# Mephisto405/WCMC

Hardware: AMD Instinct MI355X
Metric: 128x128 MC patches/sec (train step), KPCN-Manifold (higher is better)
Workload: dtype bf16x321h

## Files before the change

### include/wcmc_hip.h

```cpp
#ifndef WCMC_HIP_H
#define WCMC_HIP_H

#include <stddef.h>
#include <stdint.h>

#ifdef __cplusplus
extern "C" {
#endif

#define WCMC_ABI_VERSION 2

enum wcmc_status {
  WCMC_OK = 0,
  WCMC_ERR_BAD_ARG = -1,
  WCMC_ERR_ALIGNMENT = -2,
  WCMC_ERR_WORKSPACE = -3,
  WCMC_ERR_LAUNCH = -4
};

enum wcmc_act { WCMC_ACT_LINEAR = 0, WCMC_ACT_RELU = 1, WCMC_ACT_LEAKY_RELU = 2 };

int wcmc_abi_version(void);
const char* wcmc_last_error(void);

// ... 76 lines not shown
int wcmc_embed3_mean_fwd(const void* x_split, int64_t M, int Cin, const void* wp0, const float* b0, const void* wp1,
                         const float* b1, const void* wp2, const float* b2, float* y, float* y_mean, int S, int64_t HW,
                         void* stream);
int wcmc_embed3_bwd(const void* x_split, int64_t M, int Cin, const void* wp0, const float* b0, const void* wp1,
                    const float* b1, const void* wt1, const void* wt2, const float* gy, int gy_pixel_stride,
                    const float* gm, int gm_pixel_stride, int S, int64_t HW, float gm_scale, float* dw0, float* db0,
                    float* dw1, float* db1, float* dw2, float* db2, void* workspace, size_t workspace_bytes, void* stream);
int wcmc_final2_supported(int C1, int C2, int Chid, int outc, int64_t HW);
size_t wcmc_final2_bwd_workspace_bytes(void);
int wcmc_final2_fwd(const float* y, int y_pixel_stride, const float* prop, int prop_pixel_stride, int B, int S, int64_t HW,
                    const void* wp0, const float* b0, const void* wp1, const float* b1, int outc, float* out, void* stream);
int wcmc_final2_bwd(const float* y, int y_pixel_stride, const float* prop, int prop_pixel_stride, int B, int S, int64_t HW,
                    const void* wp0, const float* b0, const void* wp1, const float* b1, int outc, const void* wt0,
                    const void* wt1, const float* gout, float* dy, float* dprop, float* dw0, float* db0, float* dw1,
                    float* db1, void* workspace, size_t workspace_bytes, void* stream);
size_t wcmc_conv2d_igemm_colsum_elems(int N, int Ho, int Wo, int Cout);
int wcmc_colsum_finish(const float* partial, int N, int Ho, int Wo, int Cout, float* db, void* stream);
int wcmc_conv2d_launch_plan_bf16x3(int N, int H, int W, int Cin, int Cout, int ks, int pad, int terms, int split_out,
                                   int64_t ysn, int64_t ysh, int64_t ysw, int gate_tensor, int out_f16,
                                   char* cls, char* kernel, size_t len);
int wcmc_conv2d_wgrad_launch_plan_bf16x3(int N, int H, int W, int Cin, int Cout, int ks, int pad, int terms,
                                         char* cls, char* kernel, size_t len);
size_t wcmc_conv2d_wgrad_bf16x3_workspace_bytes(int N, int Ho, int Wo, int Cout, int Cin, int ks);
int wcmc_conv2d_wgrad_reduce_multi(int n, void* const* workspace, float* const* dw, float* const* db,
                                   const float* const* dy_colsum_partial, const int* N, const int* Ho, const int* Wo,
                                   const int* Cout, const int* Cin, const int* ks, int terms, void* stream);
int wcmc_conv2d_wgrad_bf16x3(const void* x_split, int N, int H, int W, int Cin,
                             const void* dy_split, int Cout, int ks, int pad, float* dw, float* db,
                             void* workspace, size_t workspace_bytes, int phase, const float* dy_colsum_partial,
                             int terms, void* stream);
// ... 233 lines not shown
```

### wcmc_amd/_lib.py

```python
import ctypes
import os

_HERE = os.path.dirname(os.path.abspath(__file__))
LIB_PATH = os.path.join(_HERE, "libwcmc_hip.so")
if os.environ.get("WCMC_DEBUG_LIB") == "1":
    LIB_PATH = os.path.join(_HERE, "libwcmc_hip_debug.so")
if os.environ.get("WCMC_LIB_AB"):
    LIB_PATH = os.path.join(_HERE, os.path.basename(os.environ["WCMC_LIB_AB"]))

_c = ctypes
P, I, L, F, D, Z = _c.c_void_p, _c.c_int, _c.c_int64, _c.c_float, _c.c_double, _c.c_size_t

SIGNATURES = {
    "wcmc_abi_version": (I, []),
    "wcmc_last_error": (_c.c_char_p, []),
    "wcmc_to_nhwc": (I, [P, L, L, L, L, P, L, L, L, I, I, I, I, P]),
    "wcmc_from_nhwc": (I, [P, L, L, L, P, L, L, L, L, I, I, I, I, P]),
    "wcmc_conv2d_packed_elems": (Z, [I, I, I]),
    "wcmc_conv2d_pack_weight": (I, [P, P, I, I, I, I, P]),
    "wcmc_conv2d_igemm": (I, [P, L, L, L, I, I, I, I, P, P, P, L, L, L, I, I, I, I, F,
                              P, L, L, L, I, F, P]),
    "wcmc_conv2d_wgrad_workspace_bytes": (Z, [I, I, I, I, I, I]),
    "wcmc_conv2d_wgrad": (I, [P, L, L, L, I, I, I, I, P, L, L, L, I, I, I, P, P, P, Z, P]),
    "wcmc_split_elems": (Z, [I, I, I, I]),
# ... 47 lines not shown
    "wcmc_pbuffer_cat_fwd": (I, [P, L, L, L, L, P, L, L, L, L, L, P, L, L, L, I, I, I, I, I, I, P]),
    "wcmc_pbuffer_cat_bwd": (I, [P, L, L, L, P, L, L, L, L, L, I, I, I, I, I, I, P]),
    "wcmc_feature_mse_workspace_bytes": (Z, [I, I, I, I, I]),
    "wcmc_feature_mse_fwd": (I, [P, L, L, L, L, L, P, L, L, L, L, P, P, P, P, Z, I, I, I, I, I, P]),
    "wcmc_feature_mse_bwd": (I, [P, L, L, L, L, L, P, P, P, P, P, Z, I, I, I, I, I, P]),
    "wcmc_grs_fwd": (I, [P, L, L, L, L, L, P, L, L, L, L, P, P, F, P, P, Z, I, I, I, I, I, P]),
    "wcmc_grs_bwd": (I, [P, L, L, L, L, L, P, P, P, P, P, Z, I, I, I, I, I, P]),
    "wcmc_random_permutation": (I, [P, L, ctypes.c_uint64, P]),
    "wcmc_permutation_key": (ctypes.c_uint64, [ctypes.c_uint64, ctypes.c_uint64, I]),
    "wcmc_random_permutation_dev": (I, [P, L, P, I, P]),
    "wcmc_step_counter_advance": (I, [P, P]),
    "wcmc_final2_supported": (I, [I, I, I, I, L]),
    "wcmc_final2_bwd_workspace_bytes": (Z, []),
    "wcmc_final2_fwd": (I, [P, I, P, I, I, I, L, P, P, P, P, I, P, P]),
    "wcmc_final2_bwd": (I, [P, I, P, I, I, I, L, P, P, P, P, I, P, P, P, P, P, P, P, P, P, P, Z, P]),
    "wcmc_embed3_supported": (I, [I, I, I, I]),
    "wcmc_embed3_bwd_workspace_bytes": (Z, []),
    "wcmc_embed3_fwd": (I, [P, L, I, P, P, P, P, P, P, P, P]),
    "wcmc_embed3_mean_supported": (I, [I, L]),
    "wcmc_embed3_mean_fwd": (I, [P, L, I, P, P, P, P, P, P, P, P, I, L, P]),
    "wcmc_embed3_bwd": (I, [P, L, I, P, P, P, P, P, P, P, I, P, I, I, L, F, P, P, P, P, P, P, P, Z, P]),
    "wcmc_image_loss2_fwd": (I, [I, P, L, L, L, L, P, L, L, L, L, F, P, P, Z, I, I, I, I, P]),
    "wcmc_image_loss2_bwd": (I, [I, P, L, L, L, L, P, L, L, L, L, F, P, P, I, I, I, I, P]),
    "wcmc_grad_norm_clip_workspace_bytes": (Z, [I, P]),
    "wcmc_grad_norm_clip": (I, [I, P, P, F, P, P, Z, P]),
    "wcmc_weight_norm_fwd": (I, [I, P, P, P, P, P, P, P]),
    "wcmc_weight_norm_bwd": (I, [I, P, P, P, P, P, P, P, P, P]),
    "wcmc_clip_adam": (I, [P, P, P, P, L, F, D, D, D, D, I, F, P, P]),
    "wcmc_clip_adam_hyper": (None, [D, D, D, D, I, P]),
    "wcmc_clip_adam_dev": (I, [P, P, P, P, L, F, F, P, P, P]),
# ... 61 lines not shown
```

### wcmc_amd/csrc/pathnet_fused.hip

```cpp
#include <stdlib.h>

#include "common.h"

namespace wcmc {

typedef __bf16 bf16x8 __attribute__((ext_vector_type(8)));
typedef unsigned short u16;
typedef short s16x4 __attribute__((ext_vector_type(4)));
typedef unsigned u32x2 __attribute__((ext_vector_type(2)));
typedef unsigned u32x4 __attribute__((ext_vector_type(4)));

constexpr unsigned E3_OOB = 0x80000000u;
constexpr int E3_TP = 64;
constexpr int E3_C = 64;
constexpr int E3_RS = 80;
constexpr int E3_TILE = E3_TP * E3_RS;

__device__ __forceinline__ u16 e3_bf(float x) { return __builtin_bit_cast(u16, (__bf16)x); }
__device__ __forceinline__ float e3_f(u16 h) { return __builtin_bit_cast(float, (unsigned)h << 16); }
__device__ __forceinline__ float e3_u2f(unsigned v) { return __builtin_bit_cast(float, v); }
__device__ __forceinline__ unsigned e3_f2u(float v) { return __builtin_bit_cast(unsigned, v); }

struct E3Params {
  const u16* x; int64_t M; int Cp0, Kt0;
// ... 371 lines not shown
}

constexpr int F2_C = 128;
constexpr int F2_RS = 144;
constexpr int F2_TILE = E3_TP * F2_RS;
constexpr int F2_ORS = 48;
constexpr int F2_W1RS = 2 * 128 + 8;

struct F2Params {
  const float* y; int y_ps;
  const float* prop; int p_ps;
  int B, S; int64_t HW;
  const u16* wp0; const u16* wp1;
  const float* b0; const float* b1; int outc;
  float* out; int os;
  const u16* wt0; const u16* wt1;
  const float* gout;
  float* dy; float* dprop;
  float* ws;
  unsigned y_bytes, p_bytes, o_bytes, dy_bytes, dp_bytes;
};
constexpr int F2_WS_PER_BLOCK = F2_C * F2_C + 16 * F2_C + F2_C + 16;

struct F2W { bf16x8 h[4], l[4]; };
__device__ __forceinline__ F2W f2_load_w(const u16* wp, int row, int q) {
  F2W w;
#pragma unroll
  for (int c = 0; c < 4; ++c) {
    const u16* a = wp + (int64_t)(row * 2) * F2_C + c * 32 + q * 8;
    w.h[c] = *reinterpret_cast<const bf16x8*>(a);
// ... 60 lines not shown
  for (int i = 0; i < 4; ++i) {
    u16 hi[4], lo[4];
#pragma unroll
    for (int e = 0; e < 4; ++e) {
      const float t = acc[i][e] + b[e];
      const float v = t > 0.f ? t : 0.f;
      hi[e] = e3_bf(v);
      lo[e] = e3_bf(v - e3_f(hi[e]));
    }
    const int o = (16 * i + fr) * F2_RS + 16 * wave + 4 * q;
    *reinterpret_cast<u32x2*>(th + o) = u32x2{(unsigned)hi[0] | ((unsigned)hi[1] << 16), (unsigned)hi[2] | ((unsigned)hi[3] << 16)};
    *reinterpret_cast<u32x2*>(tl + o) = u32x2{(unsigned)lo[0] | ((unsigned)lo[1] << 16), (unsigned)lo[2] | ((unsigned)lo[3] << 16)};
  }
}

template <bool BWD>
__global__ __launch_bounds__(512, 1) void final2_kernel(F2Params p) {
  extern __shared__ __attribute__((aligned(16))) u16 lds[];
  u16* const CH = lds; u16* const CL = lds + F2_TILE; u16* const HH = lds + 2 * F2_TILE; u16* const HL = lds + 3 * F2_TILE;
  u16* const DHH = lds + 4 * F2_TILE;
  u16* const DOH = lds + 5 * F2_TILE;
  float* const stg = reinterpret_cast<float*>(HL);
  float* const red = reinterpret_cast<float*>(lds + 5 * F2_TILE + E3_TP * F2_ORS);
  const int tid = threadIdx.x, lane = tid & 63, wave = tid >> 6, fr = lane & 15, q = lane >> 4;
  const __amdgpu_buffer_rsrc_t yr = __builtin_amdgcn_make_buffer_rsrc((void*)p.y, 0, (int)p.y_bytes, 0x00020000);
  const __amdgpu_buffer_rsrc_t pr = __builtin_amdgcn_make_buffer_rsrc((void*)p.prop, 0, (int)p.p_bytes, 0x00020000);
  const __amdgpu_buffer_rsrc_t orr = __builtin_amdgcn_make_buffer_rsrc((void*)(BWD ? (void*)p.gout : (void*)p.out), 0, (int)p.o_bytes, 0x00020000);
  u16* const W1S = reinterpret_cast<u16*>(red + 16 * F2_C + 64 * 8);
  const F2W w0 = f2_load_w(p.wp0, 16 * wave + fr, q);
  F2W w1;
  if (!BWD) w1 = f2_load_w(p.wp1, fr, q);
  float b0[4], b1[4];
#pragma unroll
  for (int e = 0; e < 4; ++e) { b0[e] = p.b0[16 * wave + 4 * q + e]; b1[e] = (4 * q + e < p.outc) ? p.b1[4 * q + e] : 0.f; }
  const int oq = p.os >> 2;
  const int64_t tpi = p.HW / E3_TP;
  const int64_t nsuper = (int64_t)p.B * tpi;

  F2W t0;
  bf16x8 t1h, t1l;
  f32x4 gw0[8], gw1;
  float sb0[4] = {0.f, 0.f, 0.f, 0.f}, sb1[4] = {0.f, 0.f, 0.f, 0.f};
// ... 20 lines not shown
    f32x4 dpacc[4];
#pragma unroll
    for (int i = 0; i < 4; ++i) dpacc[i] = f32x4{0.f, 0.f, 0.f, 0.f};
    for (int s = 0; s < p.S; ++s) {
      const int64_t m0 = (b * p.S + s) * p.HW + hw0;
      f2_store64_split(yp, CH, CL, 0, tid);
      u32x4 go = {0u, 0u, 0u, 0u};
      if (BWD && wave < 4 && q < oq)
        go = __builtin_amdgcn_raw_buffer_load_b128(orr, (unsigned)(m0 * p.os * 4) + (unsigned)((16 * wave + fr) * p.os * 4 + q * 16), 0, 0);
      if (s + 1 < p.S) yp = f2_load64(yr, (b * p.S + s + 1) * p.HW + hw0, p.y_ps, tid);
      __syncthreads();
      f32x4 acc[4];
      f2_gemm<3, 4>(acc, w0, CH, CL, 0, fr, q);
      f2_store_relu_split(acc, b0, HH, HL, wave, fr, q);
      __syncthreads();
      float ov[4] = {0.f, 0.f, 0.f, 0.f};
      if (wave < 4) {
        f32x4 a2[1];
        if (BWD) {
          a2[0] = f32x4{0.f, 0.f, 0.f, 0.f};
#pragma unroll
          for (int c = 0; c < 4; ++c) {
            const int o = (16 * wave + fr) * F2_RS + c * 32 + q * 8;
            const bf16x8 ah = *reinterpret_cast<const bf16x8*>(HH + o), al = *reinterpret_cast<const bf16x8*>(HL + o);
            const bf16x8 wh = *reinterpret_cast<const bf16x8*>(W1S + fr * F2_W1RS + c * 32 + q * 8);
            const bf16x8 wl = *reinterpret_cast<const bf16x8*>(W1S + fr * F2_W1RS + F2_C + c * 32 + q * 8);
            a2[0] = __builtin_amdgcn_mfma_f32_16x16x32_bf16(wl, ah, a2[0], 0, 0, 0);
            a2[0] = __builtin_amdgcn_mfma_f32_16x16x32_bf16(wh, al, a2[0], 0, 0, 0);
            a2[0] = __builtin_amdgcn_mfma_f32_16x16x32_bf16(wh, ah, a2[0], 0, 0, 0);
          }
// ... 65 lines not shown
        const int v = tid + 512 * k, px = v >> 4, c4 = (v & 15) * 4;
        const float4 o = *reinterpret_cast<const float4*>(stg + px * 68 + c4);
        const u32x4 o4 = {__builtin_bit_cast(unsigned, o.x), __builtin_bit_cast(unsigned, o.y), __builtin_bit_cast(unsigned, o.z),
                          __builtin_bit_cast(unsigned, o.w)};
        __builtin_amdgcn_raw_buffer_store_b128(o4, dyr, (unsigned)(m0 * 256) + (unsigned)(px * 256 + c4 * 4), 0, 0);
      }
    }
    if (BWD && wave >= 4) {
#pragma unroll
      for (int i = 0; i < 4; ++i) {
        const u32x4 o4 = {e3_f2u(dpacc[i][0]), e3_f2u(dpacc[i][1]), e3_f2u(dpacc[i][2]), e3_f2u(dpacc[i][3])};
        __builtin_amdgcn_raw_buffer_store_b128(o4, dpr, (unsigned)((b * p.HW + hw0) * 256) + (unsigned)((16 * i + fr) * 256 + (16 * (wave - 4) + 4 * q) * 4), 0, 0);
      }
    }
  }
  if (!BWD) return;
  float* ws = p.ws + (int64_t)blockIdx.x * F2_WS_PER_BLOCK;
#pragma unroll
  for (int j = 0; j < 8; ++j)
#pragma unroll
    for (int e = 0; e < 4; ++e) ws[(16 * wave + 4 * q + e) * F2_C + 16 * j + fr] = gw0[j][e];
#pragma unroll
  for (int e = 0; e < 4; ++e) ws[F2_C * F2_C + (4 * q + e) * F2_C + 16 * wave + fr] = gw1[e];
  __syncthreads();
  float* redb = red;
#pragma unroll
  for (int e = 0; e < 4; ++e) redb[fr * F2_C + 16 * wave + 4 * q + e] = sb0[e];
  if (wave < 4 && q < 2) {
#pragma unroll
    for (int e = 0; e < 4; ++e) redb[16 * F2_C + (16 * wave + fr) * 8 + 4 * q + e] = sb1[e];
  }
  __syncthreads();
  if (tid < F2_C) {
    float sacc = 0.f;
#pragma unroll
    for (int r = 0; r < 16; ++r) sacc += redb[r * F2_C + tid];
    ws[F2_C * F2_C + 16 * F2_C + tid] = sacc;
  } else if (tid < F2_C + 16) {
    const int c = tid - F2_C;
    float sacc = 0.f;
    if (c < 8)
      for (int r = 0; r < 64; ++r) sacc += redb[16 * F2_C + r * 8 + c];
    ws[F2_C * F2_C + 16 * F2_C + F2_C + c] = sacc;
  }
}

__global__ __launch_bounds__(256) void final2_bwd_finish_kernel(const float* __restrict__ ws, int nblk, int outc, float* __restrict__ dw0,
                                                                float* __restrict__ db0, float* __restrict__ dw1, float* __restrict__ db1) {
  const int i = blockIdx.x * 256 + threadIdx.x;
  if (i >= F2_WS_PER_BLOCK) return;
  float a[8] = {0.f, 0.f, 0.f, 0.f, 0.f, 0.f, 0.f, 0.f};
  int b = 0;
  for (; b + 8 <= nblk; b += 8) {
#pragma unroll
    for (int u = 0; u < 8; ++u) a[u] += ws[(int64_t)(b + u) * F2_WS_PER_BLOCK + i];
  }
  for (; b < nblk; ++b) a[0] += ws[(int64_t)b * F2_WS_PER_BLOCK + i];
  const float s = ((a[0] + a[1]) + (a[2] + a[3])) + ((a[4] + a[5]) + (a[6] + a[7]));
  if (i < F2_C * F2_C) dw0[i] = s;
  else if (i < F2_C * F2_C + 16 * F2_C) {
// ... 140 lines not shown
          u32x4 o4;
#pragma unroll
          for (int e = 0; e < 4; ++e) { const float t = a2[i][e] + b1[e]; o4[e] = e3_f2u((4 * q + e < p.outc && t > 0.f) ? t : 0.f); }
          __builtin_amdgcn_raw_buffer_store_b128(o4, orr, (unsigned)(m0 * p.os * 4) + (unsigned)((16 * i + fr) * p.os * 4 + q * 16), 0, 0);
        }
      }
    }
  }
}
constexpr size_t F2W_LDS_FWD = (size_t)(F2_C + 16) * F2W_RS * sizeof(u16) + (size_t)F2_C * sizeof(float);

static int f2_grid() { return 256; }
constexpr size_t F2_LDS_FWD = (size_t)4 * F2_TILE * sizeof(u16);
constexpr size_t F2_LDS_BWD = (size_t)5 * F2_TILE * sizeof(u16) + (size_t)E3_TP * F2_ORS * sizeof(u16) + (size_t)(16 * F2_C + 64 * 8) * sizeof(float) +
                              (size_t)16 * F2_W1RS * sizeof(u16);

static int e3_grid_bwd() { return 256; }

}

using namespace wcmc;

extern "C" int wcmc_embed3_supported(int Cin, int C1, int C2, int C3) {
  return Cin >= 1 && Cin <= 64 && C1 == 64 && C2 == 64 && C3 == 64;
}

extern "C" size_t wcmc_embed3_bwd_workspace_bytes(void) { return (size_t)e3_grid_bwd() * E3_WS_PER_BLOCK * sizeof(float); }

static int e3_fill(E3Params& p, const void* x_split, int64_t M, int Cin, const void* wp0, const float* b0, const void* wp1,
                   const float* b1) {
// ... 74 lines not shown
static int f2_fill(F2Params& p, const float* y, int y_ps, const float* prop, int p_ps, int B, int S, int64_t HW, const void* wp0,
                   const float* b0, const void* wp1, const float* b1, int outc) {
  WCMC_REQUIRE(y && prop && wp0 && wp1 && b0 && b1 && B > 0 && S > 0 && wcmc_final2_supported(64, 64, 128, outc, HW), WCMC_ERR_BAD_ARG,
               "final2: bad argument (64 + 64 -> 128 -> <= 8 channels, H*W a multiple of 64)");
  WCMC_REQUIRE(aligned16(y) && aligned16(prop) && aligned16(wp0) && aligned16(wp1) && y_ps >= 64 && y_ps % 4 == 0 && p_ps >= 64 && p_ps % 4 == 0,
               WCMC_ERR_ALIGNMENT, "final2: views must be 16-byte aligned with pixel strides that are multiples of 4 floats");
  p.y = y; p.y_ps = y_ps; p.prop = prop; p.p_ps = p_ps; p.B = B; p.S = S; p.HW = HW;
  p.wp0 = (const u16*)wp0; p.wp1 = (const u16*)wp1; p.b0 = b0; p.b1 = b1; p.outc = outc; p.os = outc <= 4 ? 4 : 8;
  const int64_t M = (int64_t)B * S * HW;
  const int64_t yb = ((M - 1) * y_ps + 64) * 4, pb = (((int64_t)B * HW - 1) * p_ps + 64) * 4, ob = M * p.os * 4;
  WCMC_REQUIRE(yb < 0x7ff00000ll && pb < 0x7ff00000ll && M * 256 < 0x7ff00000ll, WCMC_ERR_BAD_ARG, "final2: more than 2 GiB per tensor");
  p.y_bytes = (unsigned)yb; p.p_bytes = (unsigned)pb; p.o_bytes = (unsigned)ob;
  return 0;
}

extern "C" int wcmc_final2_fwd(const float* y, int y_pixel_stride, const float* prop, int prop_pixel_stride, int B, int S, int64_t HW,
                               const void* wp0, const float* b0, const void* wp1, const float* b1, int outc, float* out, void* stream) {
  F2Params p = {};
  if (int rc = f2_fill(p, y, y_pixel_stride, prop, prop_pixel_stride, B, S, HW, wp0, b0, wp1, b1, outc)) return rc;
  WCMC_REQUIRE(out && aligned16(out), WCMC_ERR_BAD_ARG, "final2_fwd: bad output");
  p.out = out;
  {
    const char* e = ab_env("WCMC_F2W");
    if (e && e[0] != '0') {
      const int ni = e[0] == '2' ? 2 : 1;
      static LdsAttr attrw1, attrw2;
      if (set_max_lds(ni == 2 ? reinterpret_cast<const void*>(&final2w_fwd_kernel<2>) : reinterpret_cast<const void*>(&final2w_fwd_kernel<1>),
                      (size_t)F2W_LDS_FWD, ni == 2 ? attrw2 : attrw1) != hipSuccess) return WCMC_ERR_LAUNCH;
      const int64_t nunits = (int64_t)B * (HW / (16 * ni)), nb = (nunits + 7) / 8;
      const int cap = ni == 2 ? f2_grid() : 2 * f2_grid();
      if (ni == 2) hipLaunchKernelGGL(final2w_fwd_kernel<2>, dim3((unsigned)(nb < cap ? nb : cap)), dim3(512), F2W_LDS_FWD, (hipStream_t)stream, p);
      else hipLaunchKernelGGL(final2w_fwd_kernel<1>, dim3((unsigned)(nb < cap ? nb : cap)), dim3(512), F2W_LDS_FWD, (hipStream_t)stream, p);
      return check_launch("final2_fwd (wave-private)");
    }
  }
  static LdsAttr attr;
  if (set_max_lds(reinterpret_cast<const void*>(&final2_kernel<false>), (size_t)F2_LDS_FWD, attr) != hipSuccess) return WCMC_ERR_LAUNCH;
  const int64_t nsuper = (int64_t)B * (HW / 64);
  hipLaunchKernelGGL(final2_kernel<false>, dim3((unsigned)(nsuper < f2_grid() ? nsuper : f2_grid())), dim3(512), F2_LDS_FWD, (hipStream_t)stream, p);
  return check_launch("final2_fwd");
}

extern "C" int wcmc_final2_bwd(const float* y, int y_pixel_stride, const float* prop, int prop_pixel_stride, int B, int S, int64_t HW,
                               const void* wp0, const float* b0, const void* wp1, const float* b1, int outc, const void* wt0,
                               const void* wt1, const float* gout, float* dy, float* dprop, float* dw0, float* db0, float* dw1,
                               float* db1, void* workspace, size_t workspace_bytes, void* stream) {
  F2Params p = {};
  if (int rc = f2_fill(p, y, y_pixel_stride, prop, prop_pixel_stride, B, S, HW, wp0, b0, wp1, b1, outc)) return rc;
  WCMC_REQUIRE(wt0 && wt1 && gout && dy && dprop && dw0 && db0 && dw1 && db1 && workspace && aligned16(wt0) && aligned16(wt1) &&
                   aligned16(gout) && aligned16(dy) && aligned16(dprop) && aligned16(workspace),
               WCMC_ERR_BAD_ARG, "final2_bwd: bad argument");
  WCMC_REQUIRE(workspace_bytes >= wcmc_final2_bwd_workspace_bytes(), WCMC_ERR_WORKSPACE, "final2_bwd: workspace too small");
  p.wt0 = (const u16*)wt0; p.wt1 = (const u16*)wt1; p.gout = gout; p.dy = dy; p.dprop = dprop; p.ws = (float*)workspace;
  const int64_t M = (int64_t)B * S * HW;
  p.dy_bytes = (unsigned)(M * 256); p.dp_bytes = (unsigned)((int64_t)B * HW * 256);
  static LdsAttr attr;
  if (set_max_lds(reinterpret_cast<const void*>(&final2_kernel<true>), (size_t)F2_LDS_BWD, attr) != hipSuccess) return WCMC_ERR_LAUNCH;
  const int nblk = f2_grid();
  hipLaunchKernelGGL(final2_kernel<true>, dim3((unsigned)nblk), dim3(512), F2_LDS_BWD, (hipStream_t)stream, p);
  if (int rc = check_launch("final2_bwd")) return rc;
  hipLaunchKernelGGL(final2_bwd_finish_kernel, dim3((unsigned)((F2_WS_PER_BLOCK + 255) / 256)), dim3(256), 0, (hipStream_t)stream,
                     (const float*)workspace, nblk, outc, dw0, db0, dw1, db1);
  return check_launch("final2_bwd_finish");
}
```

### wcmc_amd/ops/__init__.py

```python
import os

import torch
import weakref

from .._lib import check, lib

MODES = ("bf16x321h", "bf16x321", "bf16x321o", "bf16x3", "fp32")


PRECISION = os.environ.get("WCMC_PRECISION", MODES[0])
assert PRECISION in MODES, PRECISION


def _side_stream_default(mode):
    return os.environ.get("WCMC_SIDE_STREAM") == "1"


USE_SIDE_STREAM = _side_stream_default(PRECISION)

USE_BRANCH_STREAM = os.environ.get("WCMC_BRANCH_STREAM", "1") != "0"

FUSE_EMBED = os.environ.get("WCMC_FUSE_EMBED", "1") != "0"

FUSE_FINAL = os.environ.get("WCMC_FUSE_FINAL", "1") != "0"

TERMS_BY_KS = {}

EMULATE_HIDDEN = None

DEBUG_ACTS = None

DEFER_MAX_BYTES = 24 << 20

_PROFILER = None
_DEFERRED = None


def reduced_backward(mode=None):
    return (PRECISION if mode is None else mode) in ("bf16x321h", "bf16x321o", "bf16x321")
# ... 66 lines not shown
```

### wcmc_amd/ops/pathnet_fused.py

```python
import torch

from .. import ops as _sw
from .._lib import check, lib
from ._base import _Timed, _as_nhwc_nograd, _need_cuda, _ptr, _stream, _v, as_nhwc, is_nhwc_view, nhwc_empty, to_nhwc_raw
from .conv_split import (_CatBroadcastChainX, _CatUpsampleChainX, _ChainSppMeanX, _pack_chain_x, _split_shared,
                         conv_chain)
from .elementwise import cat_broadcast, spp_mean, upsample2
from .grads import _sink


def _dense_pixel_stride(g):
    n, c, h, w = g.shape
    sn, sc, sh, sw = g.stride()
    if sc == 1 and sw >= c and sw % 4 == 0 and sh == w * sw and (n == 1 or sn == h * sh) and g.data_ptr() % 16 == 0:
        return sw
    return None


class _EmbedSppMeanFusedX(torch.autograd.Function):

    @staticmethod
    def forward(ctx, x, s, *params):
        _need_cuda(x, *params)
        xs = _split_shared(x)
# ... 41 lines not shown
                  "embed3_bwd")
        return (None, None, dw0, db0, dw1, db1, dw2, db2)


class _FinalFusedX(torch.autograd.Function):

    @staticmethod
    def forward(ctx, flat, prop, s, *params):
        _need_cuda(flat, prop, *params)
        bs, c1, h, w = flat.shape
        b = prop.shape[0]
        outc = params[2].shape[0]
        packs = _pack_chain_x([params[0], params[2]], 1)
        osz = 4 if outc <= 4 else 8
        buf = torch.empty((bs, h, w, osz), device=flat.device, dtype=torch.float32)
        with _Timed("final2_fwd", 4.0 * bs * h * w * (64 + 64 // s + osz), "byte"):
            check(lib().wcmc_final2_fwd(_ptr(flat), _dense_pixel_stride(flat), _ptr(prop), _dense_pixel_stride(prop), b, s, h * w,
                                        _ptr(packs[0][0]), _ptr(params[1].detach()), _ptr(packs[1][0]), _ptr(params[3].detach()), outc,
                                        _ptr(buf), _stream()), "final2_fwd")
        ctx.geom, ctx.packs = (b, s, h, w, outc), packs
        ctx.save_for_backward(flat, prop, *params)
        return buf.permute(0, 3, 1, 2)[:, :outc]

    @staticmethod
    def backward(ctx, g):
        b, s, h, w, outc = ctx.geom
        flat, prop, w0, b0, w1, b1 = ctx.saved_tensors
        g = _as_nhwc_nograd(g)
        osz = 4 if outc <= 4 else 8
        if not (_dense_pixel_stride(g) == osz):
            g = to_nhwc_raw(g)
        dev = flat.device
        dy = torch.empty((b * s, h, w, 64), device=dev, dtype=torch.float32).permute(0, 3, 1, 2)
        dprop = nhwc_empty(b, 64, h, w, dev)
        sk = lambda t: _sink(t.data_ptr() if isinstance(t, torch.nn.Parameter) else 0, t.shape, dev)
        dw0, dw1, db0, db1 = sk(w0), sk(w1), sk(b0), sk(b1)
        nb = lib().wcmc_final2_bwd_workspace_bytes()
        ws = torch.empty(nb // 4, device=dev, dtype=torch.float32)
        packs = ctx.packs
        with _Timed("final2_bwd", 4.0 * b * s * h * w * (64 + 64 // s + osz + 64 + 64 // s), "byte"):
            check(lib().wcmc_final2_bwd(_ptr(flat), _dense_pixel_stride(flat), _ptr(prop), _dense_pixel_stride(prop), b, s, h * w,
                                        _ptr(packs[0][0]), _ptr(b0), _ptr(packs[1][0]), _ptr(b1), outc, _ptr(packs[0][1]), _ptr(packs[1][1]),
                                        _ptr(g), _ptr(dy), _ptr(dprop), _ptr(dw0), _ptr(db0), _ptr(dw1), _ptr(db1), _ptr(ws), nb,
                                        _stream()), "final2_bwd")
        return (dy if ctx.needs_input_grad[0] else None, dprop if ctx.needs_input_grad[1] else None, None, dw0, db0, dw1, db1)


_UNFUSED_NOTED = set()


def _note_unfused(what, why):
    if (what, why) not in _UNFUSED_NOTED:
        _UNFUSED_NOTED.add((what, why))
        import warnings
        warnings.warn("wcmc_amd: %s runs layer by layer (no fused kernel for %s)" % (what, why), RuntimeWarning, stacklevel=3)


def conv_chain_spp_mean(x, s, ksize, pad, acts, params):
    if (_sw.FUSE_EMBED and _sw.DEBUG_ACTS is None and ksize == 1 and pad == 0 and len(acts) == 3 and
# ... 40 lines not shown
```

Baseline: 739.3.

## Save final-head hidden activations in forward to skip backward recompute

```diff
diff --git a/include/wcmc_hip.h b/include/wcmc_hip.h
--- a/include/wcmc_hip.h
+++ b/include/wcmc_hip.h
@@ -114,6 +114,13 @@
                     const void* wp0, const float* b0, const void* wp1, const float* b1, int outc, const void* wt0,
                     const void* wt1, const float* gout, float* dy, float* dprop, float* dw0, float* db0, float* dw1,
                     float* db1, void* workspace, size_t workspace_bytes, void* stream);
+int wcmc_final2_fwd_save(const float* y, int y_pixel_stride, const float* prop, int prop_pixel_stride, int B, int S, int64_t HW,
+                         const void* wp0, const float* b0, const void* wp1, const float* b1, int outc, float* out, void* h_hi,
+                         void* stream);
+int wcmc_final2_bwd_saved(const float* y, int y_pixel_stride, const float* prop, int prop_pixel_stride, int B, int S, int64_t HW,
+                          const void* wp0, const float* b0, const void* wp1, const float* b1, int outc, const void* wt0,
+                          const void* wt1, const float* gout, const float* out, const void* h_hi, float* dy, float* dprop,
+                          float* dw0, float* db0, float* dw1, float* db1, void* workspace, size_t workspace_bytes, void* stream);
 size_t wcmc_conv2d_igemm_colsum_elems(int N, int Ho, int Wo, int Cout);
 int wcmc_colsum_finish(const float* partial, int N, int Ho, int Wo, int Cout, float* db, void* stream);
 int wcmc_conv2d_launch_plan_bf16x3(int N, int H, int W, int Cin, int Cout, int ks, int pad, int terms, int split_out,
diff --git a/wcmc_amd/_lib.py b/wcmc_amd/_lib.py
--- a/wcmc_amd/_lib.py
+++ b/wcmc_amd/_lib.py
@@ -85,6 +85,8 @@
     "wcmc_final2_bwd_workspace_bytes": (Z, []),
     "wcmc_final2_fwd": (I, [P, I, P, I, I, I, L, P, P, P, P, I, P, P]),
     "wcmc_final2_bwd": (I, [P, I, P, I, I, I, L, P, P, P, P, I, P, P, P, P, P, P, P, P, P, P, Z, P]),
+    "wcmc_final2_fwd_save": (I, [P, I, P, I, I, I, L, P, P, P, P, I, P, P, P]),
+    "wcmc_final2_bwd_saved": (I, [P, I, P, I, I, I, L, P, P, P, P, I, P, P, P, P, P, P, P, P, P, P, P, P, Z, P]),
     "wcmc_embed3_supported": (I, [I, I, I, I]),
     "wcmc_embed3_bwd_workspace_bytes": (Z, []),
     "wcmc_embed3_fwd": (I, [P, L, I, P, P, P, P, P, P, P, P]),
diff --git a/wcmc_amd/csrc/pathnet_fused.hip b/wcmc_amd/csrc/pathnet_fused.hip
--- a/wcmc_amd/csrc/pathnet_fused.hip
+++ b/wcmc_amd/csrc/pathnet_fused.hip
@@ -409,6 +409,7 @@
   const u16* wp0; const u16* wp1;
   const float* b0; const float* b1; int outc;
   float* out; int os;
+  u16* hsave; unsigned h_bytes;
   const u16* wt0; const u16* wt1;
   const float* gout;
   float* dy; float* dprop;
@@ -499,8 +500,75 @@
   }
 }
 
+__device__ __forceinline__ void f2_store64_hi(const F2Pre& o, u16* th, int c0, int tid) {
+#pragma unroll
+  for (int k = 0; k < 2; ++k) {
+    const int v = tid + 512 * k, px = v >> 4, c4 = (v & 15) * 4;
+    u16 hi[4];
+#pragma unroll
+    for (int e = 0; e < 4; ++e) hi[e] = e3_bf(e3_u2f(o.v[k][e]));
+    *reinterpret_cast<u32x2*>(th + px * F2_RS + c0 + c4) = u32x2{(unsigned)hi[0] | ((unsigned)hi[1] << 16), (unsigned)hi[2] | ((unsigned)hi[3] << 16)};
+  }
+}
+__device__ __forceinline__ void f2_save_h(const u16* th, const __amdgpu_buffer_rsrc_t r, int64_t m0, int tid) {
+  const unsigned base = (unsigned)(m0 * 256);
+#pragma unroll
+  for (int k = 0; k < 2; ++k) {
+    const int v = tid + 512 * k, px = v >> 4, u = v & 15;
+    __builtin_amdgcn_raw_buffer_store_b128(*reinterpret_cast<const u32x4*>(th + px * F2_RS + u * 8), r, base + (unsigned)(px * 256 + u * 16), 0, 0);
+  }
+}
+__device__ __forceinline__ F2Pre f2_load_h(const __amdgpu_buffer_rsrc_t r, int64_t m0, int tid) {
+  F2Pre o;
+  const unsigned base = (unsigned)(m0 * 256);
+#pragma unroll
+  for (int k = 0; k < 2; ++k) {
+    const int v = tid + 512 * k, px = v >> 4, u = v & 15;
+    o.v[k] = __builtin_amdgcn_raw_buffer_load_b128(r, base + (unsigned)(px * 256 + u * 16), 0, 0);
+  }
+  return o;
+}
+__device__ __forceinline__ void f2_store_h(const F2Pre& o, u16* th, int tid) {
+#pragma unroll
+  for (int k = 0; k < 2; ++k) {
+    const int v = tid + 512 * k, px = v >> 4, u = v & 15;
+    *reinterpret_cast<u32x4*>(th + px * F2_RS + u * 8) = o.v[k];
+  }
+}
+
+__device__ __forceinline__ void f2_bwd_partials(float* ws, float* redb, const f32x4 (&gw0)[8], const f32x4& gw1, const float (&sb0)[4],
+                                                const float (&sb1)[4], int tid) {
+  const int lane = tid & 63, wave = tid >> 6, fr = lane & 15, q = lane >> 4;
+#pragma unroll
+  for (int j = 0; j < 8; ++j)
+#pragma unroll
+    for (int e = 0; e < 4; ++e) ws[(16 * wave + 4 * q + e) * F2_C + 16 * j + fr] = gw0[j][e];
+#pragma unroll
+  for (int e = 0; e < 4; ++e) ws[F2_C * F2_C + (4 * q + e) * F2_C + 16 * wave + fr] = gw1[e];
+  __syncthreads();
+#pragma unroll
+  for (int e = 0; e < 4; ++e) redb[fr * F2_C + 16 * wave + 4 * q + e] = sb0[e];
+  if (wave < 4 && q < 2) {
+#pragma unroll
+    for (int e = 0; e < 4; ++e) redb[16 * F2_C + (16 * wave + fr) * 8 + 4 * q + e] = sb1[e];
+  }
+  __syncthreads();
+  if (tid < F2_C) {
+    float sacc = 0.f;
+#pragma unroll
+    for (int r = 0; r < 16; ++r) sacc += redb[r * F2_C + tid];
+    ws[F2_C * F2_C + 16 * F2_C + tid] = sacc;
+  } else if (tid < F2_C + 16) {
+    const int c = tid - F2_C;
+    float sacc = 0.f;
+    if (c < 8)
+      for (int r = 0; r < 64; ++r) sacc += redb[16 * F2_C + r * 8 + c];
+    ws[F2_C * F2_C + 16 * F2_C + F2_C + c] = sacc;
+  }
+}
+
 template <bool BWD>
-__global__ __launch_bounds__(512, 1) void final2_kernel(F2Params p) {
+__device__ __forceinline__ void f2_chain(const F2Params& p) {
   extern __shared__ __attribute__((aligned(16))) u16 lds[];
   u16* const CH = lds; u16* const CL = lds + F2_TILE; u16* const HH = lds + 2 * F2_TILE; u16* const HL = lds + 3 * F2_TILE;
   u16* const DHH = lds + 4 * F2_TILE;
@@ -511,6 +579,7 @@
   const __amdgpu_buffer_rsrc_t yr = __builtin_amdgcn_make_buffer_rsrc((void*)p.y, 0, (int)p.y_bytes, 0x00020000);
   const __amdgpu_buffer_rsrc_t pr = __builtin_amdgcn_make_buffer_rsrc((void*)p.prop, 0, (int)p.p_bytes, 0x00020000);
   const __amdgpu_buffer_rsrc_t orr = __builtin_amdgcn_make_buffer_rsrc((void*)(BWD ? (void*)p.gout : (void*)p.out), 0, (int)p.o_bytes, 0x00020000);
+  const __amdgpu_buffer_rsrc_t hr = __builtin_amdgcn_make_buffer_rsrc((void*)p.hsave, 0, (int)p.h_bytes, 0x00020000);
   u16* const W1S = reinterpret_cast<u16*>(red + 16 * F2_C + 64 * 8);
   const F2W w0 = f2_load_w(p.wp0, 16 * wave + fr, q);
   F2W w1;
@@ -561,6 +630,7 @@
       f2_gemm<3, 4>(acc, w0, CH, CL, 0, fr, q);
       f2_store_relu_split(acc, b0, HH, HL, wave, fr, q);
       __syncthreads();
+      if (!BWD && p.hsave) f2_save_h(HH, hr, m0, tid);
       float ov[4] = {0.f, 0.f, 0.f, 0.f};
       if (wave < 4) {
         f32x4 a2[1];
@@ -656,36 +726,141 @@
       }
     }
   }
-  if (!BWD) return;
-  float* ws = p.ws + (int64_t)blockIdx.x * F2_WS_PER_BLOCK;
-#pragma unroll
-  for (int j = 0; j < 8; ++j)
-#pragma unroll
-    for (int e = 0; e < 4; ++e) ws[(16 * wave + 4 * q + e) * F2_C + 16 * j + fr] = gw0[j][e];
-#pragma unroll
-  for (int e = 0; e < 4; ++e) ws[F2_C * F2_C + (4 * q + e) * F2_C + 16 * wave + fr] = gw1[e];
-  __syncthreads();
-  float* redb = red;
-#pragma unroll
-  for (int e = 0; e < 4; ++e) redb[fr * F2_C + 16 * wave + 4 * q + e] = sb0[e];
-  if (wave < 4 && q < 2) {
-#pragma unroll
-    for (int e = 0; e < 4; ++e) redb[16 * F2_C + (16 * wave + fr) * 8 + 4 * q + e] = sb1[e];
-  }
-  __syncthreads();
-  if (tid < F2_C) {
-    float sacc = 0.f;
-#pragma unroll
-    for (int r = 0; r < 16; ++r) sacc += redb[r * F2_C + tid];
-    ws[F2_C * F2_C + 16 * F2_C + tid] = sacc;
-  } else if (tid < F2_C + 16) {
-    const int c = tid - F2_C;
-    float sacc = 0.f;
-    if (c < 8)
-      for (int r = 0; r < 64; ++r) sacc += redb[16 * F2_C + r * 8 + c];
-    ws[F2_C * F2_C + 16 * F2_C + F2_C + c] = sacc;
-  }
-}
+  if (BWD) f2_bwd_partials(p.ws + (int64_t)blockIdx.x * F2_WS_PER_BLOCK, red, gw0, gw1, sb0, sb1, tid);
+}
+
+__device__ __forceinline__ void f2_bwd_saved(const F2Params& p) {
+  extern __shared__ __attribute__((aligned(16))) u16 lds[];
+  u16* const CH = lds; u16* const HH = lds + F2_TILE;
+  u16* const DHH = lds + 2 * F2_TILE;
+  float* const stg = reinterpret_cast<float*>(lds + 3 * F2_TILE);
+  u16* const DOH = lds + 4 * F2_TILE;
+  float* const red = reinterpret_cast<float*>(lds + 4 * F2_TILE + E3_TP * F2_ORS);
+  const int tid = threadIdx.x, lane = tid & 63, wave = tid >> 6, fr = lane & 15, q = lane >> 4;
+  const __amdgpu_buffer_rsrc_t yr = __builtin_amdgcn_make_buffer_rsrc((void*)p.y, 0, (int)p.y_bytes, 0x00020000);
+  const __amdgpu_buffer_rsrc_t pr = __builtin_amdgcn_make_buffer_rsrc((void*)p.prop, 0, (int)p.p_bytes, 0x00020000);
+  const __amdgpu_buffer_rsrc_t gr = __builtin_amdgcn_make_buffer_rsrc((void*)p.gout, 0, (int)p.o_bytes, 0x00020000);
+  const __amdgpu_buffer_rsrc_t sr = __builtin_amdgcn_make_buffer_rsrc((void*)p.out, 0, (int)p.o_bytes, 0x00020000);
+  const __amdgpu_buffer_rsrc_t hr = __builtin_amdgcn_make_buffer_rsrc((void*)p.hsave, 0, (int)p.h_bytes, 0x00020000);
+  const __amdgpu_buffer_rsrc_t dyr = __builtin_amdgcn_make_buffer_rsrc((void*)p.dy, 0, (int)p.dy_bytes, 0x00020000);
+  const __amdgpu_buffer_rsrc_t dpr = __builtin_amdgcn_make_buffer_rsrc((void*)p.dprop, 0, (int)p.dp_bytes, 0x00020000);
+  const int oq = p.os >> 2;
+  const int64_t tpi = p.HW / E3_TP;
+  const int64_t nsuper = (int64_t)p.B * tpi;
+  const bool od = wave < 4 && q < oq;
+  const unsigned oo = (unsigned)((16 * wave + fr) * p.os * 4 + q * 16);
+
+  const F2W t0 = f2_load_w(p.wt0, 16 * wave + fr, q);
+  const u16* a1 = p.wt1 + (int64_t)((16 * wave + fr) * 2) * 32 + q * 8;
+  const bf16x8 t1h = *reinterpret_cast<const bf16x8*>(a1), t1l = *reinterpret_cast<const bf16x8*>(a1 + 32);
+  f32x4 gw0[8], gw1 = f32x4{0.f, 0.f, 0.f, 0.f};
+#pragma unroll
+  for (int j = 0; j < 8; ++j) gw0[j] = f32x4{0.f, 0.f, 0.f, 0.f};
+  float sb0[4] = {0.f, 0.f, 0.f, 0.f}, sb1[4] = {0.f, 0.f, 0.f, 0.f};
+  for (int i = tid; i < E3_TP * F2_ORS / 2; i += 512) reinterpret_cast<unsigned*>(DOH)[i] = 0u;
+
+  for (int64_t st = blockIdx.x; st < nsuper; st += gridDim.x) {
+    const int64_t b = st / tpi, hw0 = (st - b * tpi) * E3_TP;
+    int64_t m0 = (b * p.S) * p.HW + hw0;
+    F2Pre pp = f2_load64(pr, b * p.HW + hw0, p.p_ps, tid);
+    F2Pre yp = f2_load64(yr, m0, p.y_ps, tid);
+    F2Pre hp = f2_load_h(hr, m0, tid);
+    u32x4 go = {0u, 0u, 0u, 0u}, so = {0u, 0u, 0u, 0u};
+    if (od) {
+      go = __builtin_amdgcn_raw_buffer_load_b128(gr, (unsigned)(m0 * p.os * 4) + oo, 0, 0);
+      so = __builtin_amdgcn_raw_buffer_load_b128(sr, (unsigned)(m0 * p.os * 4) + oo, 0, 0);
+    }
+    __syncthreads();
+    f2_store64_hi(pp, CH, 64, tid);
+    f32x4 dpacc[4];
+#pragma unroll
+    for (int i = 0; i < 4; ++i) dpacc[i] = f32x4{0.f, 0.f, 0.f, 0.f};
+    for (int s = 0; s < p.S; ++s, m0 += p.HW) {
+      f2_store64_hi(yp, CH, 0, tid);
+      f2_store_h(hp, HH, tid);
+      if (od) {
+        u16 hi[4];
+#pragma unroll
+        for (int e = 0; e < 4; ++e) {
+          const float d = e3_u2f(so[e]) > 0.f ? e3_u2f(go[e]) : 0.f;
+          sb1[e] += d;
+          hi[e] = e3_bf(d);
+        }
+        *reinterpret_cast<u32x2*>(DOH + (16 * wave + fr) * F2_ORS + 4 * q) = u32x2{(unsigned)hi[0] | ((unsigned)hi[1] << 16), (unsigned)hi[2] | ((unsigned)hi[3] << 16)};
+      }
+      if (s + 1 < p.S) {
+        const int64_t m1 = m0 + p.HW;
+        yp = f2_load64(yr, m1, p.y_ps, tid);
+        hp = f2_load_h(hr, m1, tid);
+        if (od) {
+          go = __builtin_amdgcn_raw_buffer_load_b128(gr, (unsigned)(m1 * p.os * 4) + oo, 0, 0);
+          so = __builtin_amdgcn_raw_buffer_load_b128(sr, (unsigned)(m1 * p.os * 4) + oo, 0, 0);
+        }
+      }
+      __syncthreads();
+#pragma unroll
+      for (int i = 0; i < 4; ++i) {
+        const bf16x8 dof = *reinterpret_cast<const bf16x8*>(DOH + (16 * i + fr) * F2_ORS + q * 8);
+        f32x4 a = f32x4{0.f, 0.f, 0.f, 0.f};
+        a = __builtin_amdgcn_mfma_f32_16x16x32_bf16(t1l, dof, a, 0, 0, 0);
+        a = __builtin_amdgcn_mfma_f32_16x16x32_bf16(t1h, dof, a, 0, 0, 0);
+        const int o = (16 * i + fr) * F2_RS + 16 * wave + 4 * q;
+        const u32x2 hm = *reinterpret_cast<const u32x2*>(HH + o);
+        u16 hi[4];
+#pragma unroll
+        for (int e = 0; e < 4; ++e) {
+          const u16 hv = (u16)((e < 2 ? hm[0] : hm[1]) >> (16 * (e & 1)));
+          const float d = e3_f(hv) > 0.f ? a[e] : 0.f;
+          sb0[e] += d;
+          hi[e] = e3_bf(d);
+        }
+        *reinterpret_cast<u32x2*>(DHH + o) = u32x2{(unsigned)hi[0] | ((unsigned)hi[1] << 16), (unsigned)hi[2] | ((unsigned)hi[3] << 16)};
+      }
+      __syncthreads();
+      f32x4 acc[4];
+      f2_gemm<2, 4>(acc, t0, DHH, nullptr, 0, fr, q);
+      if (wave < 4) {
+#pragma unroll
+        for (int i = 0; i < 4; ++i)
+          *reinterpret_cast<float4*>(stg + (16 * i + fr) * 68 + 16 * wave + 4 * q) = make_float4(acc[i][0], acc[i][1], acc[i][2], acc[i][3]);
+      } else {
+#pragma unroll
+        for (int i = 0; i < 4; ++i) dpacc[i] += acc[i];
+      }
+#pragma unroll
+      for (int kk = 0; kk < 2; ++kk) {
+        const bf16x8 a0 = f2_tr(DHH, F2_RS, kk, wave, lane);
+#pragma unroll
+        for (int j = 0; j < 8; ++j) gw0[j] = __builtin_amdgcn_mfma_f32_16x16x32_bf16(a0, f2_tr(CH, F2_RS, kk, j, lane), gw0[j], 0, 0, 0);
+        gw1 = __builtin_amdgcn_mfma_f32_16x16x32_bf16(f2_tr(DOH, F2_ORS, kk, 0, lane), f2_tr(HH, F2_RS, kk, wave, lane), gw1, 0, 0, 0);
+      }
+      __syncthreads();
+#pragma unroll
+      for (int k = 0; k < 2; ++k) {
+        const int v = tid + 512 * k, px = v >> 4, c4 = (v & 15) * 4;
+        const float4 o = *reinterpret_cast<const float4*>(stg + px * 68 + c4);
+        const u32x4 o4 = {__builtin_bit_cast(unsigned, o.x), __builtin_bit_cast(unsigned, o.y), __builtin_bit_cast(unsigned, o.z),
+                          __builtin_bit_cast(unsigned, o.w)};
+        __builtin_amdgcn_raw_buffer_store_b128(o4, dyr, (unsigned)(m0 * 256) + (unsigned)(px * 256 + c4 * 4), 0, 0);
+      }
+    }
+    if (wave >= 4) {
+#pragma unroll
+      for (int i = 0; i < 4; ++i) {
+        const u32x4 o4 = {e3_f2u(dpacc[i][0]), e3_f2u(dpacc[i][1]), e3_f2u(dpacc[i][2]), e3_f2u(dpacc[i][3])};
+        __builtin_amdgcn_raw_buffer_store_b128(o4, dpr, (unsigned)((b * p.HW + hw0) * 256) + (unsigned)((16 * i + fr) * 256 + (16 * (wave - 4) + 4 * q) * 4), 0, 0);
+      }
+    }
+  }
+  f2_bwd_partials(p.ws + (int64_t)blockIdx.x * F2_WS_PER_BLOCK, red, gw0, gw1, sb0, sb1, tid);
+}
+
+template <bool BWD>
+__global__ __launch_bounds__(512, 1) void final2_kernel(F2Params p) {
+  if (BWD) f2_bwd_saved(p);
+  else f2_chain<false>(p);
+}
+__global__ __launch_bounds__(512, 1) void final2_recompute_bwd_kernel(F2Params p) { f2_chain<true>(p); }
 
 __global__ __launch_bounds__(256) void final2_bwd_finish_kernel(const float* __restrict__ ws, int nblk, int outc, float* __restrict__ dw0,
                                                                 float* __restrict__ db0, float* __restrict__ dw1, float* __restrict__ db1) {
@@ -856,6 +1031,8 @@
 constexpr size_t F2_LDS_FWD = (size_t)4 * F2_TILE * sizeof(u16);
 constexpr size_t F2_LDS_BWD = (size_t)5 * F2_TILE * sizeof(u16) + (size_t)E3_TP * F2_ORS * sizeof(u16) + (size_t)(16 * F2_C + 64 * 8) * sizeof(float) +
                               (size_t)16 * F2_W1RS * sizeof(u16);
+constexpr size_t F2_LDS_BWD_SAVED = (size_t)4 * F2_TILE * sizeof(u16) + (size_t)E3_TP * F2_ORS * sizeof(u16) + (size_t)(16 * F2_C + 64 * 8) * sizeof(float);
+static_assert((size_t)E3_TP * 68 * sizeof(float) <= (size_t)F2_TILE * sizeof(u16), "the d_y staging tile fits a tile plane");
 
 static int e3_grid_bwd() { return 256; }
 
@@ -960,13 +1137,17 @@
   return 0;
 }
 
-extern "C" int wcmc_final2_fwd(const float* y, int y_pixel_stride, const float* prop, int prop_pixel_stride, int B, int S, int64_t HW,
-                               const void* wp0, const float* b0, const void* wp1, const float* b1, int outc, float* out, void* stream) {
+static int f2_fwd(const float* y, int y_pixel_stride, const float* prop, int prop_pixel_stride, int B, int S, int64_t HW, const void* wp0,
+                  const float* b0, const void* wp1, const float* b1, int outc, float* out, bool save, void* h_hi, void* stream) {
   F2Params p = {};
   if (int rc = f2_fill(p, y, y_pixel_stride, prop, prop_pixel_stride, B, S, HW, wp0, b0, wp1, b1, outc)) return rc;
   WCMC_REQUIRE(out && aligned16(out), WCMC_ERR_BAD_ARG, "final2_fwd: bad output");
   p.out = out;
-  {
+  if (save) {
+    WCMC_REQUIRE(h_hi, WCMC_ERR_BAD_ARG, "final2_fwd_save: null h_hi");
+    WCMC_REQUIRE(aligned16(h_hi), WCMC_ERR_ALIGNMENT, "final2_fwd_save: h_hi must be 16-byte aligned");
+    p.hsave = (u16*)h_hi; p.h_bytes = (unsigned)((int64_t)B * S * HW * 256);
+  } else {
     const char* e = ab_env("WCMC_F2W");
     if (e && e[0] != '0') {
       const int ni = e[0] == '2' ? 2 : 1;
@@ -987,25 +1168,61 @@
   return check_launch("final2_fwd");
 }
 
-extern "C" int wcmc_final2_bwd(const float* y, int y_pixel_stride, const float* prop, int prop_pixel_stride, int B, int S, int64_t HW,
-                               const void* wp0, const float* b0, const void* wp1, const float* b1, int outc, const void* wt0,
-                               const void* wt1, const float* gout, float* dy, float* dprop, float* dw0, float* db0, float* dw1,
-                               float* db1, void* workspace, size_t workspace_bytes, void* stream) {
+extern "C" int wcmc_final2_fwd(const float* y, int y_pixel_stride, const float* prop, int prop_pixel_stride, int B, int S, int64_t HW,
+                               const void* wp0, const float* b0, const void* wp1, const float* b1, int outc, float* out, void* stream) {
+  return f2_fwd(y, y_pixel_stride, prop, prop_pixel_stride, B, S, HW, wp0, b0, wp1, b1, outc, out, false, nullptr, stream);
+}
+extern "C" int wcmc_final2_fwd_save(const float* y, int y_pixel_stride, const float* prop, int prop_pixel_stride, int B, int S, int64_t HW,
+                                    const void* wp0, const float* b0, const void* wp1, const float* b1, int outc, float* out, void* h_hi,
+                                    void* stream) {
+  return f2_fwd(y, y_pixel_stride, prop, prop_pixel_stride, B, S, HW, wp0, b0, wp1, b1, outc, out, true, h_hi, stream);
+}
+
+static int f2_bwd(const float* y, int y_pixel_stride, const float* prop, int prop_pixel_stride, int B, int S, int64_t HW,
+                  const void* wp0, const float* b0, const void* wp1, const float* b1, int outc, const void* wt0,
+                  const void* wt1, const float* gout, bool saved, const float* out, const void* h_hi, float* dy, float* dprop, float* dw0,
+                  float* db0, float* dw1, float* db1, void* workspace, size_t workspace_bytes, void* stream) {
   F2Params p = {};
   if (int rc = f2_fill(p, y, y_pixel_stride, prop, prop_pixel_stride, B, S, HW, wp0, b0, wp1, b1, outc)) return rc;
   WCMC_REQUIRE(wt0 && wt1 && gout && dy && dprop && dw0 && db0 && dw1 && db1 && workspace && aligned16(wt0) && aligned16(wt1) &&
                    aligned16(gout) && aligned16(dy) && aligned16(dprop) && aligned16(workspace),
                WCMC_ERR_BAD_ARG, "final2_bwd: bad argument");
+  if (saved) {
+    WCMC_REQUIRE(out && h_hi, WCMC_ERR_BAD_ARG, "final2_bwd_saved: null out or h_hi");
+    WCMC_REQUIRE(aligned16(out) && aligned16(h_hi), WCMC_ERR_ALIGNMENT, "final2_bwd_saved: out and h_hi must be 16-byte aligned");
+  }
   WCMC_REQUIRE(workspace_bytes >= wcmc_final2_bwd_workspace_bytes(), WCMC_ERR_WORKSPACE, "final2_bwd: workspace too small");
   p.wt0 = (const u16*)wt0; p.wt1 = (const u16*)wt1; p.gout = gout; p.dy = dy; p.dprop = dprop; p.ws = (float*)workspace;
   const int64_t M = (int64_t)B * S * HW;
   p.dy_bytes = (unsigned)(M * 256); p.dp_bytes = (unsigned)((int64_t)B * HW * 256);
-  static LdsAttr attr;
-  if (set_max_lds(reinterpret_cast<const void*>(&final2_kernel<true>), (size_t)F2_LDS_BWD, attr) != hipSuccess) return WCMC_ERR_LAUNCH;
   const int nblk = f2_grid();
-  hipLaunchKernelGGL(final2_kernel<true>, dim3((unsigned)nblk), dim3(512), F2_LDS_BWD, (hipStream_t)stream, p);
+  if (saved) {
+    p.out = const_cast<float*>(out); p.hsave = (u16*)const_cast<void*>(h_hi); p.h_bytes = (unsigned)(M * 256);
+    static LdsAttr attrs;
+    if (set_max_lds(reinterpret_cast<const void*>(&final2_kernel<true>), (size_t)F2_LDS_BWD_SAVED, attrs) != hipSuccess) return WCMC_ERR_LAUNCH;
+    hipLaunchKernelGGL(final2_kernel<true>, dim3((unsigned)nblk), dim3(512), F2_LDS_BWD_SAVED, (hipStream_t)stream, p);
+  } else {
+    static LdsAttr attr;
+    if (set_max_lds(reinterpret_cast<const void*>(&final2_recompute_bwd_kernel), (size_t)F2_LDS_BWD, attr) != hipSuccess) return WCMC_ERR_LAUNCH;
+    hipLaunchKernelGGL(final2_recompute_bwd_kernel, dim3((unsigned)nblk), dim3(512), F2_LDS_BWD, (hipStream_t)stream, p);
+  }
   if (int rc = check_launch("final2_bwd")) return rc;
   hipLaunchKernelGGL(final2_bwd_finish_kernel, dim3((unsigned)((F2_WS_PER_BLOCK + 255) / 256)), dim3(256), 0, (hipStream_t)stream,
                      (const float*)workspace, nblk, outc, dw0, db0, dw1, db1);
   return check_launch("final2_bwd_finish");
 }
+
+extern "C" int wcmc_final2_bwd(const float* y, int y_pixel_stride, const float* prop, int prop_pixel_stride, int B, int S, int64_t HW,
+                               const void* wp0, const float* b0, const void* wp1, const float* b1, int outc, const void* wt0,
+                               const void* wt1, const float* gout, float* dy, float* dprop, float* dw0, float* db0, float* dw1,
+                               float* db1, void* workspace, size_t workspace_bytes, void* stream) {
+  return f2_bwd(y, y_pixel_stride, prop, prop_pixel_stride, B, S, HW, wp0, b0, wp1, b1, outc, wt0, wt1, gout, false, nullptr, nullptr, dy, dprop,
+                dw0, db0, dw1, db1, workspace, workspace_bytes, stream);
+}
+extern "C" int wcmc_final2_bwd_saved(const float* y, int y_pixel_stride, const float* prop, int prop_pixel_stride, int B, int S, int64_t HW,
+                                     const void* wp0, const float* b0, const void* wp1, const float* b1, int outc, const void* wt0,
+                                     const void* wt1, const float* gout, const float* out, const void* h_hi, float* dy, float* dprop,
+                                     float* dw0, float* db0, float* dw1, float* db1, void* workspace, size_t workspace_bytes, void* stream) {
+  return f2_bwd(y, y_pixel_stride, prop, prop_pixel_stride, B, S, HW, wp0, b0, wp1, b1, outc, wt0, wt1, gout, true, out, h_hi, dy, dprop,
+                dw0, db0, dw1, db1, workspace, workspace_bytes, stream);
+}
diff --git a/wcmc_amd/ops/__init__.py b/wcmc_amd/ops/__init__.py
--- a/wcmc_amd/ops/__init__.py
+++ b/wcmc_amd/ops/__init__.py
@@ -23,6 +23,8 @@
 FUSE_EMBED = os.environ.get("WCMC_FUSE_EMBED", "1") != "0"
 
 FUSE_FINAL = os.environ.get("WCMC_FUSE_FINAL", "1") != "0"
+
+SAVE_FINAL_HIDDEN = True
 
 TERMS_BY_KS = {}
 
diff --git a/wcmc_amd/ops/pathnet_fused.py b/wcmc_amd/ops/pathnet_fused.py
--- a/wcmc_amd/ops/pathnet_fused.py
+++ b/wcmc_amd/ops/pathnet_fused.py
@@ -79,18 +79,25 @@
         packs = _pack_chain_x([params[0], params[2]], 1)
         osz = 4 if outc <= 4 else 8
         buf = torch.empty((bs, h, w, osz), device=flat.device, dtype=torch.float32)
-        with _Timed("final2_fwd", 4.0 * bs * h * w * (64 + 64 // s + osz), "byte"):
-            check(lib().wcmc_final2_fwd(_ptr(flat), _dense_pixel_stride(flat), _ptr(prop), _dense_pixel_stride(prop), b, s, h * w,
-                                        _ptr(packs[0][0]), _ptr(params[1].detach()), _ptr(packs[1][0]), _ptr(params[3].detach()), outc,
-                                        _ptr(buf), _stream()), "final2_fwd")
+        args = (_ptr(flat), _dense_pixel_stride(flat), _ptr(prop), _dense_pixel_stride(prop), b, s, h * w,
+                _ptr(packs[0][0]), _ptr(params[1].detach()), _ptr(packs[1][0]), _ptr(params[3].detach()), outc, _ptr(buf))
+        saved = ()
+        if _sw.SAVE_FINAL_HIDDEN and any(ctx.needs_input_grad):
+            hhi = torch.empty((bs * h * w, 128), device=flat.device, dtype=torch.bfloat16)
+            with _Timed("final2_fwd", 4.0 * bs * h * w * (64 + 64 // s + osz + 64), "byte"):
+                check(lib().wcmc_final2_fwd_save(*args, _ptr(hhi), _stream()), "final2_fwd_save")
+            saved = (hhi, buf)
+        else:
+            with _Timed("final2_fwd", 4.0 * bs * h * w * (64 + 64 // s + osz), "byte"):
+                check(lib().wcmc_final2_fwd(*args, _stream()), "final2_fwd")
         ctx.geom, ctx.packs = (b, s, h, w, outc), packs
-        ctx.save_for_backward(flat, prop, *params)
+        ctx.save_for_backward(flat, prop, *params, *saved)
         return buf.permute(0, 3, 1, 2)[:, :outc]
 
     @staticmethod
     def backward(ctx, g):
         b, s, h, w, outc = ctx.geom
-        flat, prop, w0, b0, w1, b1 = ctx.saved_tensors
+        flat, prop, w0, b0, w1, b1, *saved = ctx.saved_tensors
         g = _as_nhwc_nograd(g)
         osz = 4 if outc <= 4 else 8
         if not (_dense_pixel_stride(g) == osz):
@@ -103,11 +110,16 @@
         nb = lib().wcmc_final2_bwd_workspace_bytes()
         ws = torch.empty(nb // 4, device=dev, dtype=torch.float32)
         packs = ctx.packs
-        with _Timed("final2_bwd", 4.0 * b * s * h * w * (64 + 64 // s + osz + 64 + 64 // s), "byte"):
-            check(lib().wcmc_final2_bwd(_ptr(flat), _dense_pixel_stride(flat), _ptr(prop), _dense_pixel_stride(prop), b, s, h * w,
-                                        _ptr(packs[0][0]), _ptr(b0), _ptr(packs[1][0]), _ptr(b1), outc, _ptr(packs[0][1]), _ptr(packs[1][1]),
-                                        _ptr(g), _ptr(dy), _ptr(dprop), _ptr(dw0), _ptr(db0), _ptr(dw1), _ptr(db1), _ptr(ws), nb,
-                                        _stream()), "final2_bwd")
+        ins = (_ptr(flat), _dense_pixel_stride(flat), _ptr(prop), _dense_pixel_stride(prop), b, s, h * w,
+               _ptr(packs[0][0]), _ptr(b0), _ptr(packs[1][0]), _ptr(b1), outc, _ptr(packs[0][1]), _ptr(packs[1][1]), _ptr(g))
+        outs = (_ptr(dy), _ptr(dprop), _ptr(dw0), _ptr(db0), _ptr(dw1), _ptr(db1), _ptr(ws), nb, _stream())
+        if saved:
+            hhi, buf = saved
+            with _Timed("final2_bwd", 4.0 * b * s * h * w * (64 + 64 // s + osz + 64 + 64 // s + 64 + osz), "byte"):
+                check(lib().wcmc_final2_bwd_saved(*ins, _ptr(buf), _ptr(hhi), *outs), "final2_bwd_saved")
+        else:
+            with _Timed("final2_bwd", 4.0 * b * s * h * w * (64 + 64 // s + osz + 64 + 64 // s), "byte"):
+                check(lib().wcmc_final2_bwd(*ins, *outs), "final2_bwd")
         return (dy if ctx.needs_input_grad[0] else None, dprop if ctx.needs_input_grad[1] else None, None, dw0, db0, dw1, db1)
 
 
```

Result: faster. 752.0 (median of 6 runs) (+1.7%).
